# lofcz/Infidex

Measured on AMD Instinct MI355X. Metric: queries/sec, 10M-doc corpus, top-k=20 (whole hot path, index resident in HBM), higher is better.
Workload: dtype f32; 1 GPU; BASELINE config 4: 10000000 docs, vocab 1000000, 1 field(s), 1000-query batches, 2-3-word queries 30% fuzzed, depth 500, top-20; docs=10000000, batch=1000, top_k=20, coverage_depth=500, sessions_in_flight=4, parallelism=single GPU

## Files before the change

### infidex_amd/csrc/infidex_hip.hip

```cpp
#include <type_traits>
#include <cstring>
#include <hip/hip_runtime.h>
#include <stdint.h>
#include <string.h>
#include <stdio.h>
#include <string>
#include <vector>
#include <unordered_map>
#include <algorithm>
#include <map>
#include <mutex>
#include <chrono>
#include <thread>
#include <dlfcn.h>
#include <rccl/rccl.h>
#include "../../include/infidex_hip.h"
#include "unicode_tables.h"

#define WAVE 64
#define FILT_MAXCOL 64

static thread_local std::string g_err;
static int32_t fail(int32_t code, const char* fmt, const char* a = "") {
    char buf[512]; snprintf(buf, sizeof buf, fmt, a); g_err = buf; return code;
}
#define HIPCHK(x) do { hipError_t e_ = (x); if (e_ != hipSuccess) return fail(INFX_EHIP, #x ": %s", hipGetErrorString(e_)); } while (0)
static inline hipError_t enter_device(int device) { const hipError_t e = hipSetDevice(device); (void)hipGetLastError(); return e; }

struct DevIndex {
    int32_t N, T, R, rshift, nRanges, docBase, totalDocs;
    const uint64_t* postOff; const int32_t* postDoc; const uint8_t* postW;
    const float* docNorm;
    const float* docLen;
    const uint8_t* deleted;
    const int64_t* docKey;
    const uint64_t* textOff; const uint16_t* text;
    const uint32_t* skipIdx;
    const uint32_t* skipTbl;
    const uint32_t* psSkip;
    const uint32_t* psSkipTbl;
    const int32_t* wmExact;
    const int32_t* wmLd1;
    const int64_t* docKeyAll;
    int packed;
// ... 483 lines not shown
static hipError_t lds_limit(const void* fn, int device, size_t lds) {
    if (lds <= 64 * 1024) return hipSuccess;
    static std::mutex mu; static std::map<std::pair<int, const void*>, size_t> mark;
    std::lock_guard<std::mutex> lk(mu);
    size_t& hw = mark[{device, fn}];
    if (lds > hw) { const hipError_t e = hipFuncSetAttribute(fn, hipFuncAttributeMaxDynamicSharedMemorySize, (int)lds); if (e != hipSuccess) return e; hw = lds; }
    return hipSuccess;
}

template <int R> static void launch_union(infx_stream* s, uint32_t nv, const uint32_t* dBeg, const uint32_t* dEnd, const int32_t* dMembers, uint32_t* dRangeCount,
                                            const unsigned long long* dBase, int32_t* outDocs) {
    uint64_t blocks = (uint64_t)nv * s->ix->d.nRanges;
    k_union<R><<<dim3((unsigned)blocks), dim3(WAVE), 0, s->st>>>(dev_index(s), dBeg, dEnd, dMembers, nv, dRangeCount, dBase, outDocs);
}
static void launch_union_any(infx_stream* s, uint32_t nv, const uint32_t* dBeg, const uint32_t* dEnd, const int32_t* dMembers, uint32_t* dRangeCount,
                             const unsigned long long* dBase, int32_t* outDocs) {
    switch (s->ix->d.R) {
        case 512: launch_union<512>(s, nv, dBeg, dEnd, dMembers, dRangeCount, dBase, outDocs); break;
        case 1024: launch_union<1024>(s, nv, dBeg, dEnd, dMembers, dRangeCount, dBase, outDocs); break;
        case 2048: launch_union<2048>(s, nv, dBeg, dEnd, dMembers, dRangeCount, dBase, outDocs); break;
        case 4096: launch_union<4096>(s, nv, dBeg, dEnd, dMembers, dRangeCount, dBase, outDocs); break;
        case 8192: launch_union<8192>(s, nv, dBeg, dEnd, dMembers, dRangeCount, dBase, outDocs); break;
        default: launch_union<16384>(s, nv, dBeg, dEnd, dMembers, dRangeCount, dBase, outDocs); break;
    }
}
static bool exact_enabled(const infx_index* ix) { static const bool v = [] { const char* e = getenv("INFX_EXACT"); return !(e && e[0] == '0'); }(); return v && !(ix->cfg.flags & INFX_CFG_NO_EXACT_REPLAY); }
static Arena make_arena(infx_stream* s) {
    return Arena{s->arDoc, s->arScore, s->arCls, s->arMask, s->arExc, (const unsigned long long*)s->dBlockOut, (uint32_t*)s->dBlockOutHi,
                 (uint32_t*)s->dCounts, s->dOverflow, (unsigned long long*)s->dQBytes, (uint32_t*)((unsigned long long*)s->dQBytes + s->lastNqAlloc), (uint2*)s->dDir, s->maskWords};
}
static int acc_stripe() { static const int v = [] { const char* e = getenv("INFX_ACC_STRIPE"); int x = e ? atoi(e) : 0; return (x >= 1 && x <= 64) ? x : 4; }(); return v; }
template <int R> static bool acc_lds_layout_ok() {
    static const bool ok = [] {
        hipFuncAttributes a1{}, a2{}, a4{};
        if (hipFuncGetAttributes(&a1, (const void*)k_accumulate<R, 1>) != hipSuccess || hipFuncGetAttributes(&a2, (const void*)k_accumulate<R, 2>) != hipSuccess ||
            hipFuncGetAttributes(&a4, (const void*)k_accumulate<R, 4>) != hipSuccess) return false;
        return a1.sharedSizeBytes == 0 && a2.sharedSizeBytes == 0 && a4.sharedSizeBytes == 0;
    }();
    return ok;
}
static int acc_sparse_t() { static const int v = [] { const char* e = getenv("INFX_ACC_SPARSE_T"); const int x = e ? atoi(e) : 96; return std::max(0, std::min(4096, x)); }(); return v; }
template <int R> static void launch_acc(infx_stream* s, uint32_t nq, Arena ar, int maxT, int useGrp, int maxRef) {
    (void)maxRef;
    if (!acc_lds_layout_ok<R>()) { s->accLayoutBad = true; return; }
    static const int dbgSkip = [] { const char* e = getenv("INFX_ACC_SKIP"); return e ? atoi(e) : 0; }();
    const int sparseT = s->ix->hPostOff.empty() || s->ix->hPostOff.back() + 4 <= 0xFFFFFFF0ull ? acc_sparse_t() : 0;
    const int stripe = sparseT > 0 ? std::max(1, std::min(4, 65536 / R)) : acc_stripe();
    const int nStripes = (s->ix->d.nRanges + stripe - 1) / stripe;
    const uint64_t blocks = (uint64_t)nq * 8u * ((nStripes + 7) / 8);
    const uint8_t* dense = nullptr;
    if (sparseT > 0) {
        if (grow(s, &s->dDense, &s->capDense, (size_t)nq * nStripes)) { s->accLayoutBad = true; return; }
        hipMemsetAsync(s->dDense, 0, (size_t)nq * nStripes, s->st);
        const size_t sw = (size_t)stripe * (R / 32);
        const int maxTl = (std::min(64, std::max(1, maxT)) + 3) & ~3;
        static const int dbgS = [] { const char* e = getenv("INFX_ACCS_SKIP"); return e ? atoi(e) : 0; }();
        const size_t ldsS = (sw + 64 + 4) * 4 + INFX_NCLASS * 4 + WAVE * 2 + WAVE * 12 + (size_t)WAVE * maxTl + (size_t)64 * maxTl;
#define ACCS_LAUNCH(MW_) k_accumulate_sparse<R, MW_><<<dim3((unsigned)blocks), dim3(WAVE), ldsS, s->st>>>(dev_index(s), (const DevQuery*)s->dQueries, (const DevTerm*)s->dTerms, (const int32_t*)s->dExtra, \
            (const int32_t*)s->dUDocs, (const uint32_t*)s->dURange, nq, ar, stripe, useGrp, (uint8_t*)s->dDense, (uint32_t)sparseT, nStripes, maxTl, dbgS)
        if (ar.maskWords == 4) ACCS_LAUNCH(4); else if (ar.maskWords == 2) ACCS_LAUNCH(2); else ACCS_LAUNCH(1);
#undef ACCS_LAUNCH
        dense = (const uint8_t*)s->dDense;
    }
    const size_t lds = (size_t)R + 128 + ((size_t)(R / 32) + 2) * 4 + INFX_NCLASS * 4 + ACC_CAP_DEFAULT * 2;
#define ACC_LAUNCH(MW_) k_accumulate<R, MW_><<<dim3((unsigned)blocks), dim3(WAVE), lds, s->st>>>(dev_index(s), (const DevQuery*)s->dQueries, (const DevTerm*)s->dTerms, (const int32_t*)s->dExtra, \
        (const int32_t*)s->dUDocs, (const uint32_t*)s->dURange, nq, ar, maxT, stripe, useGrp, dbgSkip, (unsigned long long*)s->dStats, dense, nStripes, \
        s->nAccHeavy != 0xFFFFFFFFu ? (const uint32_t*)s->dAccOrder : nullptr, s->nAccHeavy != 0xFFFFFFFFu ? s->nAccHeavy : 0u)
    if (ar.maskWords == 4) ACC_LAUNCH(4); else if (ar.maskWords == 2) ACC_LAUNCH(2); else ACC_LAUNCH(1);
#undef ACC_LAUNCH
    if (dbgSkip & 8) { unsigned long long h[4] = {0, 0, 0, 0}; hipStreamSynchronize(s->st); hipMemcpy(h, s->dStats, 32, hipMemcpyDeviceToHost); hipMemset(s->dStats, 0, 32);
        fprintf(stderr, "[infx] k_accumulate stats: %llu ranges with candidates (%llu blocks), %.2f rounds/range, %.1f candidates/range\n", h[0], (unsigned long long)blocks, h[0] ? (double)h[1] / h[0] : 0.0, h[0] ? (double)h[2] / h[0] : 0.0); }
}

static const uint32_t* select_order(infx_stream* s, uint32_t nq) {
    static const bool off = [] { const char* e = getenv("INFX_SELECT_LPT"); return e && e[0] == '0'; }();
    if (off || nq < 64 || nq > SEL_ORDER_MAX) return nullptr;
    if (grow(s, &s->dSelOrder, &s->capSelOrder, (size_t)nq * 4)) return nullptr;
    k_select_order<<<1, 1024, 0, s->st>>>((const uint32_t*)s->dBlockOutHi, nq, (uint32_t*)s->dSelOrder);
    return (const uint32_t*)s->dSelOrder;
}
#ifdef SEL_PROF
static void wgprof_dump(const char* name, const unsigned long long* dProf, uint32_t n, const char* const ph[5], hipStream_t st) {
    hipStreamSynchronize(st);
    std::vector<unsigned long long> h((size_t)n * 8); hipMemcpy(h.data(), dProf, h.size() * 8, hipMemcpyDeviceToHost);
    unsigned long long t0 = ~0ull, t5 = 0; for (uint32_t q = 0; q < n; q++) if (h[q * 8]) { t0 = std::min(t0, h[q * 8]); for (int k = 1; k < 6; k++) t5 = std::max(t5, h[q * 8 + k]); }
    fprintf(stderr, "[%s] span %.1f us\n", name, (t5 - t0) / 100.0);
    auto endOf = [&](uint32_t q) { unsigned long long e = h[q * 8]; for (int k = 1; k < 6; k++) e = std::max(e, h[q * 8 + k]); return e; };
    std::vector<uint32_t> ord(n); for (uint32_t q = 0; q < n; q++) ord[q] = q;
    std::sort(ord.begin(), ord.end(), [&](uint32_t a, uint32_t b) { return endOf(a) - h[a * 8] > endOf(b) - h[b * 8]; });
    auto us = [&](uint32_t q, int a, int b) { const unsigned long long x = h[q * 8 + a], y = h[q * 8 + b]; return (x && y) ? (double)(y - x) / 100.0 : -1.0; };
    auto line = [&](const char* tag, uint32_t q) { fprintf(stderr, "[%s] %s wg %u w6 %llu w7 %llu: start %.1f total %.1f | %s %.1f %s %.1f %s %.1f %s %.1f %s %.1f\n", name, tag, q, h[q * 8 + 6], h[q * 8 + 7], (h[q * 8] - t0) / 100.0,
                                                        (endOf(q) - h[q * 8]) / 100.0, ph[0], us(q, 0, 1), ph[1], us(q, 1, 2), ph[2], us(q, 2, 3), ph[3], us(q, 3, 4), ph[4], us(q, 4, 5)); };
    for (int i = 0; i < 10 && i < (int)n; i++) line("top", ord[i]);
    line("p50", ord[n / 2]); line("p90", ord[n / 10]); line("p99", ord[n / 100]);
    std::vector<unsigned long long> en(n); for (uint32_t q = 0; q < n; q++) en[q] = endOf(q) - t0; std::sort(en.begin(), en.end());
    fprintf(stderr, "[%s] ends: p10 %.1f p50 %.1f p90 %.1f p99 %.1f max %.1f us\n", name, en[n / 10] / 100.0, en[n / 2] / 100.0, en[n * 9 / 10] / 100.0, en[n * 99 / 100] / 100.0, en[n - 1] / 100.0);
}
#endif
static uint32_t giant_min_rows() { static const uint32_t v = [] { const char* e = getenv("INFX_SEL_GIANT_MIN"); return e ? (uint32_t)std::max(0, atoi(e)) : 65536u; }(); return v; }
static SelGiant select_giants(infx_stream* s, Arena ar, uint32_t nq, const uint32_t* order) {
    const uint32_t minRows = giant_min_rows();
    SelGiant G{}; if (!order || !minRows || !s->nBoundGiants || s->maxQueryBound < 4ull * minRows) return G;
    const size_t head = (size_t)SELG_MAX * 2 * 4096 * 4 + (size_t)SELG_MAX * 4 * 5, total = head + (size_t)SELG_MAX * SEL_CAP * 8;
    if (grow(s, &s->dSelG, &s->capSelG, total)) return G;
// ... 2376 lines not shown
```

### infidex_amd/csrc/stage1.hip.inc

```

#define F_LOWEST 0x100
#define F_S1 0x200
#define F_S2 0x400
#define CLS_HOLE 0xFF

struct Arena {
    int32_t* doc; float* score; uint8_t* cls;
    unsigned long long* mask;
    uint32_t* exc;
    const unsigned long long* qBase;
    uint32_t* qCursor;
    uint32_t* counts;
    uint32_t* overflow;
    unsigned long long* qBytes;
    uint32_t* qMax;
    uint2* dir;
    int maskWords;
};

#define ACC_WPS 4
#define ACC_PF 2
#define ACC_G 2
#define ACC_CAP_DEFAULT (64 * ACC_G)

typedef int v4i_t __attribute__((ext_vector_type(4)));
typedef const __attribute__((address_space(1))) v4i_t* gint4p;
__device__ __forceinline__ int4 ld4(gint4p p, uint32_t i) { const v4i_t v = p[i]; return make_int4(v.x, v.y, v.z, v.w); }
typedef const __attribute__((address_space(1))) int32_t* gint32p;
__device__ __forceinline__ uint32_t rdl_u(uint32_t v, int l) { return (uint32_t)__builtin_amdgcn_readlane((int)v, l); }
__device__ __forceinline__ float rdl_f(float v, int l) { return __int_as_float(__builtin_amdgcn_readlane(__float_as_int(v), l)); }

typedef __attribute__((address_space(3))) uint8_t lds_u8_t;
#define LDS8(off) (*(lds_u8_t*)(uint32_t)(off))

template <int R, int MW>
__global__ __launch_bounds__(WAVE, ACC_WPS) void k_accumulate(DevIndex ix, const DevQuery* __restrict__ queries,
                                                      const DevTerm* __restrict__ terms, const int32_t* __restrict__ extraDocs,
                                                      const int32_t* __restrict__ unionDocs, const uint32_t* __restrict__ unionRange, uint32_t nq, Arena ar, int maxT, int stripe, int useGrp, int dbgSkip, unsigned long long* __restrict__ stats,
                                                      const uint8_t* __restrict__ dense, int nStripes, const uint32_t* __restrict__ qOrder, uint32_t nHeavy) {
    constexpr int W = R / 32;
    constexpr int WPL = (W + WAVE - 1) / WAVE;
    constexpr int G = ACC_G, CAP = WAVE * ACC_G;
    extern __shared__ __attribute__((aligned(16))) unsigned char smem[];
    uint8_t* sTf = (uint8_t*)smem;
    uint32_t* sBits = (uint32_t*)(sTf + R + 128);
    uint32_t* sHist = sBits + W + 2;
    uint16_t* sDoc = (uint16_t*)(sHist + INFX_NCLASS);

    const int lane = threadIdx.x;
    const uint32_t b = blockIdx.x;
    uint32_t q; int sIdx;
    if (dbgSkip & 32) { q = b % nq; sIdx = (int)(b / nq); }
    else if (qOrder) {
        const uint32_t ns8 = (uint32_t)((nStripes + 7) / 8) * 8u, hb = nHeavy * ns8;
        if (b < hb) { q = qOrder[b / ns8]; sIdx = (int)(b % ns8); }
        else { const uint32_t t = (b - hb) >> 3, nr = nq - nHeavy; q = qOrder[nHeavy + t % nr]; sIdx = (int)((t / nr) * 8u + (b & 7u)); }
    }
    else { const uint32_t t = b >> 3; q = t % nq; sIdx = (int)((t / nq) * 8u + (b & 7u)); }
    if (sIdx * stripe >= ix.nRanges) return;
    if (dense && !dense[(size_t)q * nStripes + (size_t)sIdx]) return;
    const DevQuery Q = queries[q];
    const uint8_t* const del = q_deleted(ix, q);
    const int mode = Q.mode;
    const int nT = (int)Q.numTerms;
    const DevTerm* T = terms + Q.termOff;
    const int nAnd = Q.nAnd;
    const uint32_t Rlane = (uint32_t)R + (uint32_t)lane;
    const unsigned long long qb = ar.qBase[q];
    const uint32_t qcap = (uint32_t)(ar.qBase[q + 1] - qb);
    const int nWin = (nT + WAVE - 1) / WAVE;

    for (int i = lane * 16; i < R + 128; i += WAVE * 16) *(uint4*)(sTf + i) = make_uint4(0, 0, 0, 0);
    for (int i = lane; i < INFX_NCLASS; i += WAVE) sHist[i] = 0;
    unsigned long long myBytes = 0;
    uint32_t myMax = 0;

    uint32_t tApLo = 0, tApHi = 0, tPack = 0, tLen = 0, tMeta = 0, tUpd = 0x1FFu << 16; float tIdf = 0.f;
    uint32_t tRef = 0; bool tGen = false;
    DevTerm tm{}; bool tmValid = false;
    auto load_window_consts = [&](int win) {
        const int t = win * WAVE + lane;
        tmValid = t < nT;
        if (tmValid) tm = T[t];
        tIdf = (tmValid && tm.idf > 0.f) ? tm.idf : 0.f;
        tMeta = tmValid ? (((uint32_t)tm.isVirtual << 16) | ((uint32_t)tm.pad << 24)) : 0u;
        tUpd = 0x1FFu << 16;
        if (tmValid) {
            uint32_t add = 0, rk1 = 0x1FFu;
            if (mode == INFX_MODE_AND) add = ((tm.role & INFX_ROLE_AND) ? 1u : 0u) | ((tm.role & INFX_ROLE_LOWEST) ? F_LOWEST : 0u) | ((tm.role & INFX_ROLE_S1) ? F_S1 : 0u) | ((tm.role & INFX_ROLE_S2) ? F_S2 : 0u);
            else if (mode == INFX_MODE_DISJ && (tm.role & (INFX_ROLE_ELIGIBLE | INFX_ROLE_LOWQ))) rk1 = (uint32_t)tm.rank + 1u;
            tUpd = add | (rk1 << 16);
        }
        tRef = tmValid ? tm.refIdx : 0u;
// ... 273 lines not shown
                        if (pre) cls |= 0x80; else atomicAdd(&sHist[cls], 1u);
                    }
                } else { emit = true; cls = 1; atomicAdd(&sHist[1], 1u); }
            }
            const unsigned long long m = __ballot(emit);
            if (emit) {
                const unsigned long long pos = outBase + written + __popcll(m & ((1ull << lane) - 1));
                ar.doc[pos] = ix.docBase + base + l;
                const float stored = (del && del[ix.docBase + base + l]) ? 0.f : sc;
                ar.score[pos] = stored; myMax = max(myMax, __float_as_uint(stored));
                ar.cls[pos] = cls;
                if (ar.maskWords) {
#pragma unroll
                    for (int w = 0; w < MW; w++) ar.mask[pos * (unsigned long long)MW + w] = cMask[g][w];
                    ar.exc[pos] = cExc[g];
                }
            }
            written += (uint32_t)__popcll(m);
        }
    }
    if (!haveOff || dropped) continue;
    if (lane == 0) { ar.dir[(unsigned long long)q * ix.nRanges + r] = make_uint2(chunkOff, written); myBytes += (unsigned long long)written * 12ull; }
    for (uint32_t i = written + lane; i < ncand; i += WAVE) { ar.cls[outBase + i] = CLS_HOLE; ar.score[outBase + i] = 0.f; }
    }
    for (int i = lane; i < INFX_NCLASS; i += WAVE) { uint32_t c = sHist[i]; if (c) atomicAdd(&ar.counts[(uint64_t)q * INFX_NCLASS + i], c); }
#pragma unroll
    for (int d = 32; d > 0; d >>= 1) myBytes += __shfl_down(myBytes, d);
    if (lane == 0 && myBytes) atomicAdd(&ar.qBytes[q], myBytes);
#pragma unroll
    for (int d = 32; d > 0; d >>= 1) myMax = max(myMax, (uint32_t)__shfl_down((int)myMax, d));
    if (lane == 0 && myMax) atomicMax(&ar.qMax[q], myMax);
}

template <int R>
__global__ __launch_bounds__(WAVE) void k_union(DevIndex ix, const uint32_t* __restrict__ memberBeg, const uint32_t* __restrict__ memberEnd, const int32_t* __restrict__ members,
                                                 uint32_t nv, uint32_t* __restrict__ rangeCount, const unsigned long long* __restrict__ unionBase,
                                                 int32_t* __restrict__ outDocs) {
    constexpr int W = R / 32;
    constexpr int WPL = (W + WAVE - 1) / WAVE;
    __shared__ uint32_t sBits[W];
    __shared__ unsigned long long sBase[WAVE];
    __shared__ uint32_t sLen[WAVE];
    const int lane = threadIdx.x;
    const uint32_t v = blockIdx.x % nv; const int r = (int)(blockIdx.x / nv);
    const int32_t base = r * R, rend = min(base + R, ix.N);
    if (outDocs) { if (r + 1 <= ix.nRanges && rangeCount[(uint64_t)v * (ix.nRanges + 1) + r] == rangeCount[(uint64_t)v * (ix.nRanges + 1) + r + 1]) return; }
    for (int i = lane; i < W; i += WAVE) sBits[i] = 0;
    const uint32_t mb = memberBeg[v], me = memberEnd[v];
    bool any = false;
    for (uint32_t m0 = mb; m0 < me; m0 += WAVE) {
        uint32_t len = 0; unsigned long long b0 = 0;
        if (m0 + lane < me) {
            const int32_t t = members[m0 + lane];
            const uint64_t tb = ix.postOff[t], te = ix.postOff[t + 1];
            const uint32_t sk = ix.skipIdx[t];
            uint32_t lo, hi;
            if (sk != 0xFFFFFFFFu) { lo = ix.skipTbl[sk + r]; hi = ix.skipTbl[sk + r + 1]; }
            else { lo = (uint32_t)(lower_bound_post(ix.postDoc, tb, te, base, ix.packed) - tb); hi = (uint32_t)(lower_bound_post(ix.postDoc, tb + lo, te, rend, ix.packed) - tb); }
            len = hi - lo; b0 = tb + lo;
        }
        sBase[lane] = b0; sLen[lane] = len;
        const int nm = (int)min((uint32_t)WAVE, me - m0);
        for (int k = 0; k < nm; k++) {
            const uint32_t L = sLen[k]; const unsigned long long bb = sBase[k];
            if (L) any = true;
            for (uint32_t i = lane; i < L; i += WAVE) { int l = post_doc(ix.postDoc[bb + i], ix.packed) - base; atomicOr(&sBits[l >> 5], 1u << (l & 31)); }
// ... 393 lines not shown
```

### infidex_amd/csrc/stage1_sparse.hip.inc

```
#define ACCS_U 6

template <int R, int MW>
__global__ __launch_bounds__(WAVE) void k_accumulate_sparse(DevIndex ix, const DevQuery* __restrict__ queries, const DevTerm* __restrict__ terms, const int32_t* __restrict__ extraDocs,
                                                            const int32_t* __restrict__ unionDocs, const uint32_t* __restrict__ unionRange, uint32_t nq, Arena ar, int stripe, int useGrp,
                                                            uint8_t* __restrict__ denseFlag, uint32_t denseT, int nStripes, int maxTl, int dbg) {
    constexpr int U = ACCS_U;
    extern __shared__ __attribute__((aligned(16))) unsigned char smem[];
    const int SW = stripe * (R / 32);
    const int WPL = max(1, SW / WAVE);
    const int wsh = 31 - __clz(WPL);
    const int SWP = (SW + (SW >> wsh) + 3) & ~3;
    uint32_t* sBits = (uint32_t*)smem;
    uint32_t* sHist = sBits + SWP;
    uint16_t* sDoc = (uint16_t*)(sHist + INFX_NCLASS);
    uint2* sTA = (uint2*)(sDoc + WAVE);
    uint32_t* sTL = (uint32_t*)(sTA + WAVE);
    uint8_t* sHit = (uint8_t*)(sTL + WAVE);
    uint32_t* sSamp = (uint32_t*)(sHit + (size_t)WAVE * maxTl);

    const int lane = threadIdx.x;
    const uint32_t b = blockIdx.x;
    const uint32_t bt = b >> 3; const uint32_t q = bt % nq; const int sIdx = (int)((bt / nq) * 8u + (b & 7u));
    const int r0 = sIdx * stripe;
    if (r0 >= ix.nRanges) return;
    const int rEnd = min(ix.nRanges, r0 + stripe), nr = rEnd - r0;
    const int32_t base = r0 * R;
    const int32_t send = min(rEnd * R, ix.N);
    const uint32_t span = (uint32_t)(send - base);
    const DevQuery Q = queries[q];
    const uint8_t* const del = q_deleted(ix, q);
    const int mode = Q.mode;
    const int nT = (int)Q.numTerms;
    const DevTerm* T = terms + Q.termOff;
    const int nAnd = Q.nAnd;
    const unsigned long long qb = ar.qBase[q];
    const uint32_t qcap = (uint32_t)(ar.qBase[q + 1] - qb);
    const int nWin = (nT + WAVE - 1) / WAVE;
    const unsigned long long lt = (1ull << lane) - 1;
    unsigned long long myBytes = 0;

    uint32_t tApLo = 0, tApHi = 0, tLen = 0, tMeta = 0, tUpd = 0x1FFu << 16; float tIdf = 0.f;
    auto load_window = [&](int win) -> bool {
        const int t = win * WAVE + lane;
        tLen = 0; tApLo = 0; tApHi = 0; tIdf = 0.f; tMeta = 0; tUpd = 0x1FFu << 16;
        bool gen = false;
        if (t < nT) {
            const DevTerm tm = T[t];
            tIdf = tm.idf > 0.f ? tm.idf : 0.f;
            uint32_t add = 0, rk1 = 0x1FFu;
            if (mode == INFX_MODE_AND) {
                add = ((tm.role & INFX_ROLE_AND) ? 1u : 0u) | ((tm.role & INFX_ROLE_LOWEST) ? F_LOWEST : 0u) | ((tm.role & INFX_ROLE_S1) ? F_S1 : 0u) | ((tm.role & INFX_ROLE_S2) ? F_S2 : 0u);
                gen = (tm.role & (INFX_ROLE_S1 | INFX_ROLE_S2)) != 0;
            } else if (mode == INFX_MODE_DISJ && (tm.role & (INFX_ROLE_ELIGIBLE | INFX_ROLE_LOWQ))) { rk1 = (uint32_t)tm.rank + 1u; gen = true; }
            tUpd = add | (rk1 << 16);
            tMeta = (uint32_t)tm.isVirtual | ((uint32_t)tm.pad << 8) | ((uint32_t)tm.refIdx << 16);
            uint32_t lo, hi;
            if (tm.isVirtual & 4) { lo = unionRange[tm.skip + r0]; hi = unionRange[tm.skip + rEnd]; }
            else if (tm.skip != 0xFFFFFFFFu) { lo = ix.skipTbl[tm.skip + r0]; hi = ix.skipTbl[tm.skip + rEnd]; }
            else {
                const int32_t* arr = (tm.isVirtual & 1) ? extraDocs : ix.postDoc;
                const int pk = (tm.isVirtual & 5) ? 0 : ix.packed;
                lo = (uint32_t)(lower_bound_post(arr, tm.begin, tm.end, base, pk) - tm.begin);
                hi = (uint32_t)(lower_bound_post(arr, tm.begin + lo, tm.end, send, pk) - tm.begin);
            }
            tLen = hi - lo;
            const int32_t* dp = ((tm.isVirtual & 4) ? unionDocs : ((tm.isVirtual & 1) ? extraDocs : ix.postDoc)) + (tm.begin + lo);
            const unsigned long long ap = (unsigned long long)(uintptr_t)dp;
            tApLo = (uint32_t)ap; tApHi = (uint32_t)(ap >> 32);
            myBytes += (unsigned long long)tLen * (tm.isVirtual ? 4u : 5u);
        }
        return gen;
    };

    unsigned long long psBase = 0; uint32_t psLen = 0;
    if (Q.prefixSet >= 0) {
        const uint64_t pb = ix.psOff[Q.prefixSet], pe = ix.psOff[Q.prefixSet + 1];
        const uint32_t sk = ix.psSkip[Q.prefixSet];
        uint64_t lo, hi;
        if (sk != 0xFFFFFFFFu) { lo = pb + ix.psSkipTbl[sk + r0]; hi = pb + ix.psSkipTbl[sk + rEnd]; }
        else { lo = lower_bound_i32(ix.psDocs, pb, pe, base); hi = lower_bound_i32(ix.psDocs, lo, pe, send); }
        psBase = lo; psLen = (uint32_t)(hi - lo);
    }
    bool anyGen = (mode == INFX_MODE_PREFIX) && psLen > 0;
    bool bitsClear = false;
    auto set_bit = [&](uint32_t l) { const uint32_t w = l >> 5; atomicOr(&sBits[w + (w >> wsh)], 1u << (l & 31)); };
    auto clear_bits = [&]() { if (!bitsClear) { for (int i = lane * 4; i < SWP; i += WAVE * 4) *(uint4*)(sBits + i) = make_uint4(0, 0, 0, 0); bitsClear = true; } };
    if (mode == INFX_MODE_PREFIX) {
        if (psLen > denseT) { if (lane == 0) denseFlag[(size_t)q * nStripes + sIdx] = 1; return; }
        if (nWin == 1) load_window(0);
        if (anyGen) { clear_bits(); for (uint32_t i = lane; i < psLen; i += WAVE) set_bit((uint32_t)(ix.psDocs[psBase + i] - base)); }
    } else {
        for (int win = 0; win < nWin; win++) {
            const bool gen = load_window(win);
            if (__ballot(gen && tLen > denseT)) { if (lane == 0) denseFlag[(size_t)q * nStripes + sIdx] = 1; return; }
            unsigned long long gm = __ballot(gen && tLen > 0);
            if (gm) { anyGen = true; clear_bits(); }
            while (gm) {
                const int tl = __ffsll((long long)gm) - 1; gm &= gm - 1;
                const uint32_t len = rdl_u(tLen, tl), iv = rdl_u(tMeta, tl) & 0xFFu;
                const unsigned long long ap = ((unsigned long long)rdl_u(tApHi, tl) << 32) | rdl_u(tApLo, tl);
                const int pk = (iv & 5) ? 0 : ix.packed;
                if (!(iv & 1)) {
                    const uint32_t mis = (uint32_t)((ap >> 2) & 3u);
                    const gint4p ap4 = (gint4p)(uintptr_t)(ap - 4ull * mis);
                    const uint32_t total = len + mis;
                    for (uint32_t i = (uint32_t)lane * 4u; i < total; i += 4u * WAVE) {
                        const int4 c = ld4(ap4, i >> 2);
                        const uint32_t l0 = (uint32_t)post_doc(c.x, pk) - (uint32_t)base, l1 = (uint32_t)post_doc(c.y, pk) - (uint32_t)base;
                        const uint32_t l2 = (uint32_t)post_doc(c.z, pk) - (uint32_t)base, l3 = (uint32_t)post_doc(c.w, pk) - (uint32_t)base;
                        if (l0 < span) set_bit(l0);
                        if (l1 < span) set_bit(l1);
                        if (l2 < span) set_bit(l2);
                        if (l3 < span) set_bit(l3);
                    }
                } else {
                    const gint32p dp = (gint32p)(uintptr_t)ap;
                    for (uint32_t i = lane; i < len; i += WAVE) set_bit((uint32_t)(post_doc(dp[i], pk) - base));
                }
            }
        }
    }
    uint32_t ncand = 0, cnt = 0, incl = 0;
    if (anyGen) {
        for (int j = 0; j < WPL; j++) { const int wi = lane * WPL + j; if (wi < SW) cnt += __popc(sBits[wi + lane]); }
        incl = cnt;
#pragma unroll
        for (int d = 1; d < WAVE; d <<= 1) { const uint32_t v = __shfl_up(incl, d); if (lane >= d) incl += v; }
        ncand = rdl_u(incl, WAVE - 1);
    }
    if (ncand > denseT) {
        if (lane == 0) denseFlag[(size_t)q * nStripes + sIdx] = 1;
        return;
    }
    if (dbg & 2) ncand = 0;
    if (ncand) {
        for (int i = lane; i < INFX_NCLASS; i += WAVE) sHist[i] = 0;
        uint32_t chunkOffV = 0;
        if (lane == 0) chunkOffV = atomicAdd(&ar.qCursor[q], ncand);
        uint32_t chunkOff = 0; unsigned long long outBase = 0; bool haveOff = false, dropped = false;
        uint32_t written = 0, rCnt = 0, myMax = 0;
        for (uint32_t rb = 0; rb < ncand && !dropped; rb += WAVE) {
        const uint32_t nslot = min((uint32_t)WAVE, ncand - rb);
        {
            uint32_t sl = incl - cnt;
            if (sl < rb + nslot && incl > rb)
                for (int j = 0; j < WPL; j++) {
                    const int wi = lane * WPL + j;
                    uint32_t bits = wi < SW ? sBits[wi + lane] : 0u;
                    while (bits) { const int bpos = __ffs(bits) - 1; bits &= bits - 1; const uint32_t rel = sl - rb; if (rel < nslot) sDoc[rel] = (uint16_t)(wi * 32 + bpos); sl++; }
                }
        }
        const bool valid = (uint32_t)lane < nslot;
        const uint32_t cDoc = valid ? (uint32_t)sDoc[lane] : 0u;
        const uint32_t docS = (uint32_t)base + cDoc;
        const float cNorm = valid ? ix.docNorm[docS] : 1.0f;
        float cAcc = 0.f; uint32_t cFlag = 0, cRank = 0x1FFu, cGrp = 0, cExc = 0; unsigned long long cMask[MW];
#pragma unroll
        for (int w = 0; w < MW; w++) cMask[w] = 0ull;

        struct TermS { uint32_t meta, upd; float idf; };
        auto apply = [&](const TermS& S, uint32_t tfb) {
            const uint32_t iv = S.meta & 0xFFu, grp = (S.meta >> 8) & 0xFFu, ref = S.meta >> 16;
            const bool unit = iv != 0;
            if (!__ballot(tfb != 0)) return;
            if (grp && useGrp) { const bool dup = cGrp == grp; if (tfb) cGrp = grp; if (dup) tfb = 0; }
            const bool hit = tfb != 0;
            {
                const float tf = unit ? 1.0f : (float)tfb;
                const float denom = tf + cNorm;
                const float core = (tf * (1.2f + 1.0f)) / denom;
                const float sc = S.idf * (core + 1.0f);
                cAcc += hit ? sc : 0.f;
            }
            const uint32_t addFlag = S.upd & 0xFFFFu, rk1 = S.upd >> 16;
            cFlag += hit ? addFlag : 0u;
            cRank = min(cRank, hit ? rk1 : 0x1FFu);
            if (ar.maskWords != 0 && ref < 32u * (uint32_t)MW) {
                const uint32_t capCode = unit ? 1u : 3u;
                const unsigned long long code = (unsigned long long)min(tfb, capCode) << ((ref & 31u) * 2u);
                const uint32_t wsel = ref >> 5;
#pragma unroll
                for (int w = 0; w < MW; w++) if (wsel == (uint32_t)w) cMask[w] |= code;
                if (!unit && __ballot(tfb >= 3u)) {
                    const uint32_t rec = ((ref + 1u) << 8) | tfb;
                    if (tfb >= 3u) { if (!(cExc & 0xFFFFu)) cExc |= rec; else if (!(cExc >> 16)) cExc |= rec << 16; }
                }
            }
        };
        const uint32_t tpp = (uint32_t)WAVE / nslot;
        const uint32_t mdiv = (65536u + nslot - 1u) / nslot;
        const uint32_t kl = ((uint32_t)lane * mdiv) >> 16, cl = (uint32_t)lane - kl * nslot;
        const uint32_t pairDoc = (uint32_t)base + (uint32_t)sDoc[cl < nslot ? cl : 0];
        for (int win = 0; win < nWin; win++) {
            if (nWin > 1) load_window(win);
            const unsigned long long tmask = __ballot(tLen > 0);
            if (!tmask) continue;
            const uint32_t nLive = (uint32_t)__popcll(tmask);
            if (tLen > 0) {
                const uint32_t k = (uint32_t)__popcll(tmask & lt), iv = tMeta & 0xFFu;
                sTA[k] = make_uint2(tApLo, tApHi); sTL[k] = tLen | ((iv & 5u) ? 1u << 29 : 0u);
            }
            for (uint32_t i = (uint32_t)lane * 4u; i < nLive * (uint32_t)WAVE; i += 4u * WAVE) *(uint32_t*)(sHit + i) = 0u;
            for (uint32_t i = (uint32_t)lane; i < nLive * 16u; i += WAVE) {
                const uint32_t k = i >> 4, j = i & 15u;
                const uint2 a = sTA[k]; const uint32_t len = sTL[k] & 0x1FFFFFFFu;
                sSamp[i] = ((const uint32_t*)(uintptr_t)(((unsigned long long)a.y << 32) | a.x))[(j * len) >> 4];
            }
            const uint32_t keyP = ix.packed ? ((pairDoc << 8) | 0xFFu) : pairDoc;
            const uint32_t* const pd = (const uint32_t*)ix.postDoc;
            for (uint32_t k0 = 0; k0 < nLive && !(dbg & 1); k0 += tpp * (uint32_t)U) {
                uint32_t n[U], pos[U], xb[U];
#pragma unroll
                for (int u = 0; u < U; u++) {
                    const uint32_t kk = k0 + (uint32_t)u * tpp + kl;
                    n[u] = 0; pos[u] = 0; xb[u] = 0xFFFFFFFFu;
                    if (kl < tpp && kk < nLive) {
                        const uint32_t L = sTL[kk];
                        if (!((L >> 29) & 1u)) {
                            const uint2 a = sTA[kk];
                            const uint32_t A = (uint32_t)((const uint32_t*)(uintptr_t)(((unsigned long long)a.y << 32) | a.x) - pd), len = L & 0x1FFFFFFFu;
                            const uint32_t* sp = sSamp + kk * 16u;
                            uint32_t j = 0;
#pragma unroll
                            for (uint32_t st = 8; st > 0; st >>= 1) j += (sp[j + st] <= keyP) ? st : 0u;
                            const uint32_t lo = (j * len) >> 4, hi = j == 15u ? len : (((j + 1u) * len) >> 4);
                            pos[u] = A + lo; n[u] = max(hi - lo, 1u); xb[u] = sp[j];
                        }
                    }
                }
                bool more = false;
#pragma unroll
                for (int u = 0; u < U; u++) more = more || n[u] > 1;
                while (__ballot(more)) {
                    uint32_t o[U], x[U];
#pragma unroll
                    for (int u = 0; u < U; u++) { const uint32_t half = n[u] >> 1; o[u] = pos[u] + half; x[u] = (n[u] > 1) ? pd[o[u]] : xb[u]; n[u] -= half; }
                    more = false;
#pragma unroll
                    for (int u = 0; u < U; u++) { const bool le = x[u] <= keyP; pos[u] = le ? o[u] : pos[u]; xb[u] = le ? x[u] : xb[u]; more = more || n[u] > 1; }
                }
#pragma unroll
                for (int u = 0; u < U; u++) {
                    if (ix.packed ? (xb[u] >> 8) == pairDoc : xb[u] == pairDoc) {
                        const uint32_t tfb = ix.packed ? (xb[u] & 0xFFu) : (uint32_t)ix.postW[pos[u]];
                        sHit[(k0 + (uint32_t)u * tpp + kl) * (uint32_t)WAVE + cl] = (uint8_t)tfb;
                    }
                }
            }
            for (unsigned long long lm = (dbg & 1) ? 0ull : __ballot((uint32_t)lane < nLive && ((sTL[lane] >> 29) & 1u)); lm; lm &= lm - 1) {
                const uint32_t kL = (uint32_t)__ffsll((long long)lm) - 1u;
                const uint2 a = sTA[kL]; const uint32_t len = sTL[kL] & 0x1FFFFFFFu;
                const uint32_t* lp = (const uint32_t*)(uintptr_t)(((unsigned long long)a.y << 32) | a.x);
                if (valid) {
                    uint32_t lo = 0, hi = len;
                    while (lo < hi) { const uint32_t m = (lo + hi) >> 1; if (lp[m] < docS) lo = m + 1u; else hi = m; }
                    if (lo < len && lp[lo] == docS) sHit[kL * (uint32_t)WAVE + (uint32_t)lane] = (uint8_t)1u;
                }
            }
            uint32_t k = 0;
            for (unsigned long long tm = (dbg & 4) ? 0ull : tmask; tm; tm &= tm - 1, k++) {
                const int tl = __ffsll((long long)tm) - 1;
                TermS S; S.meta = rdl_u(tMeta, tl); S.upd = rdl_u(tUpd, tl); S.idf = rdl_f(tIdf, tl);
                apply(S, valid ? (uint32_t)sHit[k * (uint32_t)WAVE + (uint32_t)lane] : 0u);
            }
        }
        if (!haveOff) {
            chunkOff = (uint32_t)rfl_i((int)chunkOffV); haveOff = true;
            if (chunkOff + ncand > qcap) { if (lane == 0) atomicExch(ar.overflow, 1u); dropped = true; }
            outBase = qb + chunkOff;
        }
        if (!dropped) {
            bool emit = false; uint8_t cls = 0; const float sc = cAcc; const uint32_t f = (mode == INFX_MODE_DISJ) ? (cRank == 0x1FFu ? 0u : cRank) : cFlag;
            if (valid && sc > 0.f) {
                if (mode == INFX_MODE_AND) {
                    if (f & (F_S1 | F_S2)) {
                        emit = true;
                        const int c2 = (int)(f & 0xFF);
                        const bool t1 = c2 == nAnd - 1;
                        const bool t0b = t1 && (f & F_LOWEST);
                        cls = (uint8_t)((t0b ? 1 : 0) | ((t1 && nAnd >= 3) ? 2 : 0) | ((f & F_S1) ? 4 : 0) | ((f & F_S2) ? 8 : 0));
                        atomicAdd(&sHist[cls], 1u);
                    }
                } else if (mode == INFX_MODE_DISJ) {
                    if (f != 0) {
                        emit = true;
                        cls = (uint8_t)((f - 1) & 0x7F);
                        bool pre = false;
                        if (psLen) {
                            const int32_t d = (int32_t)docS;
                            const uint64_t p = lower_bound_i32(ix.psDocs, psBase, psBase + psLen, d);
                            pre = p < psBase + psLen && ix.psDocs[p] == d;
                        }
                        if (pre) cls |= 0x80; else atomicAdd(&sHist[cls], 1u);
                    }
                } else { emit = true; cls = 1; atomicAdd(&sHist[1], 1u); }
            }
            const unsigned long long m = __ballot(emit);
// ... 1 lines not shown
                const unsigned long long pos = outBase + written + __popcll(m & lt);
                ar.doc[pos] = ix.docBase + (int32_t)docS;
                const float stored = (del && del[ix.docBase + (int32_t)docS]) ? 0.f : sc;
                ar.score[pos] = stored; myMax = max(myMax, __float_as_uint(stored));
                ar.cls[pos] = cls;
                if (ar.maskWords) {
#pragma unroll
                    for (int w = 0; w < MW; w++) ar.mask[pos * (unsigned long long)MW + w] = cMask[w];
                    ar.exc[pos] = cExc;
                }
            }
            written += (uint32_t)__popcll(m);
            const uint32_t rng = cDoc / (uint32_t)R;
#pragma unroll 1
            for (int k = 0; k < nr; k++) { const uint32_t c = (uint32_t)__popcll(__ballot(emit && rng == (uint32_t)k)); if (lane == k) rCnt += c; }
        }
        }
        if (haveOff && !dropped) {
            uint32_t rIncl = rCnt;
#pragma unroll
            for (int d = 1; d < WAVE; d <<= 1) { const uint32_t v = __shfl_up(rIncl, d); if (lane >= d) rIncl += v; }
            if (lane < nr && rCnt) ar.dir[(unsigned long long)q * ix.nRanges + r0 + lane] = make_uint2(chunkOff + rIncl - rCnt, rCnt);
            if (lane == 0) myBytes += (unsigned long long)written * 12ull;
            for (uint32_t i = written + lane; i < ncand; i += WAVE) { ar.cls[outBase + i] = CLS_HOLE; ar.score[outBase + i] = 0.f; }
            for (int i = lane; i < INFX_NCLASS; i += WAVE) { const uint32_t c = sHist[i]; if (c) atomicAdd(&ar.counts[(uint64_t)q * INFX_NCLASS + i], c); }
#pragma unroll
            for (int d = 32; d > 0; d >>= 1) myMax = max(myMax, (uint32_t)__shfl_down((int)myMax, d));
            if (lane == 0 && myMax) atomicMax(&ar.qMax[q], myMax);
        }
    }
#pragma unroll
    for (int d = 32; d > 0; d >>= 1) myBytes += __shfl_down(myBytes, d);
    if (lane == 0 && myBytes) atomicAdd(&ar.qBytes[q], myBytes);
}
```

Measured before the change: 96080 queries/s.

## Merge sparse and streaming accumulate into one launch with in-block fallback

Adds k_accumulate_merged, which runs the sparse accumulation body and, when a stripe turns out dense, falls through to the streaming body in the same block. The dense-flag buffer, its memset, and the second kernel launch that re-reads it are no longer needed. The term-table LDS size is capped so occupancy matches the streaming kernel, and windows with too many live terms are handed to the streaming path. The cost is a heavier combined kernel whose register pressure could lower occupancy, plus possible extra streaming work when the cap forces a fallback. Wave barriers were also added inside the sparse body.

```diff
diff --git a/infidex_amd/csrc/infidex_hip.hip b/infidex_amd/csrc/infidex_hip.hip
--- a/infidex_amd/csrc/infidex_hip.hip
+++ b/infidex_amd/csrc/infidex_hip.hip
@@ -10,6 +10,7 @@
 #include <algorithm>
 #include <map>
 #include <mutex>
+#include <atomic>
 #include <chrono>
 #include <thread>
 #include <dlfcn.h>
@@ -559,44 +560,82 @@
 static int acc_stripe() { static const int v = [] { const char* e = getenv("INFX_ACC_STRIPE"); int x = e ? atoi(e) : 0; return (x >= 1 && x <= 64) ? x : 4; }(); return v; }
 template <int R> static bool acc_lds_layout_ok() {
     static const bool ok = [] {
-        hipFuncAttributes a1{}, a2{}, a4{};
-        if (hipFuncGetAttributes(&a1, (const void*)k_accumulate<R, 1>) != hipSuccess || hipFuncGetAttributes(&a2, (const void*)k_accumulate<R, 2>) != hipSuccess ||
-            hipFuncGetAttributes(&a4, (const void*)k_accumulate<R, 4>) != hipSuccess) return false;
-        return a1.sharedSizeBytes == 0 && a2.sharedSizeBytes == 0 && a4.sharedSizeBytes == 0;
+        const void* const k[6] = {(const void*)k_accumulate<R, 1>, (const void*)k_accumulate<R, 2>, (const void*)k_accumulate<R, 4>,
+                                  (const void*)k_accumulate_merged<R, 1>, (const void*)k_accumulate_merged<R, 2>, (const void*)k_accumulate_merged<R, 4>};
+        for (const void* f : k) { hipFuncAttributes a{}; if (hipFuncGetAttributes(&a, f) != hipSuccess || a.sharedSizeBytes != 0) return false; }
+        return true;
     }();
     return ok;
 }
 static int acc_sparse_t() { static const int v = [] { const char* e = getenv("INFX_ACC_SPARSE_T"); const int x = e ? atoi(e) : 96; return std::max(0, std::min(4096, x)); }(); return v; }
+static bool acc_merged() { static const bool v = [] { const char* e = getenv("INFX_ACC_MERGED"); return !(e && e[0] == '0'); }(); return v; }
+static size_t acc_sparse_lds(int R, int stripe, int maxTl) {
+    return ((size_t)stripe * (R / 32) + 64 + 4) * 4 + INFX_NCLASS * 4 + WAVE * 2 + WAVE * 12 + (size_t)WAVE * maxTl + (size_t)64 * maxTl;
+}
+template <int R, int MW> static int acc_merged_max_tl(int stripe, size_t ldsStream) {
+    static const int cap = [&] {
+        int nStream = 0, n = 0;
+        if (hipOccupancyMaxActiveBlocksPerMultiprocessor(&nStream, (const void*)k_accumulate<R, MW>, WAVE, ldsStream) != hipSuccess || nStream <= 0) return 0;
+        for (int tl = 64; tl >= 4; tl -= 4)
+            if (hipOccupancyMaxActiveBlocksPerMultiprocessor(&n, (const void*)k_accumulate_merged<R, MW>, WAVE, std::max(ldsStream, acc_sparse_lds(R, stripe, tl))) == hipSuccess && n >= nStream) return tl;
+        return 0;
+    }();
+    return cap;
+}
 template <int R> static void launch_acc(infx_stream* s, uint32_t nq, Arena ar, int maxT, int useGrp, int maxRef) {
     (void)maxRef;
     if (!acc_lds_layout_ok<R>()) { s->accLayoutBad = true; return; }
     static const int dbgSkip = [] { const char* e = getenv("INFX_ACC_SKIP"); return e ? atoi(e) : 0; }();
+    static const int dbgS = [] { const char* e = getenv("INFX_ACCS_SKIP"); return e ? atoi(e) : 0; }();
+    static const bool dbgPrint = getenv("INFX_DEBUG") != nullptr;
     const int sparseT = s->ix->hPostOff.empty() || s->ix->hPostOff.back() + 4 <= 0xFFFFFFF0ull ? acc_sparse_t() : 0;
     const int stripe = sparseT > 0 ? std::max(1, std::min(4, 65536 / R)) : acc_stripe();
     const int nStripes = (s->ix->d.nRanges + stripe - 1) / stripe;
     const uint64_t blocks = (uint64_t)nq * 8u * ((nStripes + 7) / 8);
+    const size_t lds = (size_t)R + 128 + ((size_t)(R / 32) + 2) * 4 + INFX_NCLASS * 4 + ACC_CAP_DEFAULT * 2;
+    const uint32_t* const qOrder = s->nAccHeavy != 0xFFFFFFFFu ? (const uint32_t*)s->dAccOrder : nullptr;
+    const uint32_t nHeavy = s->nAccHeavy != 0xFFFFFFFFu ? s->nAccHeavy : 0u;
+    const int maxTl = (std::min(64, std::max(1, maxT)) + 3) & ~3;
     const uint8_t* dense = nullptr;
-    if (sparseT > 0) {
+    int schedule = 0, tlUsed = 0;
+    if (sparseT > 0 && acc_merged() && !(dbgSkip & 32)) {
+        const int capTl = ar.maskWords == 4 ? acc_merged_max_tl<R, 4>(stripe, lds) : ar.maskWords == 2 ? acc_merged_max_tl<R, 2>(stripe, lds) : acc_merged_max_tl<R, 1>(stripe, lds);
+        if (capTl > 0) {
+            schedule = 1; tlUsed = std::min(maxTl, capTl);
+            const size_t ldsM = std::max(lds, acc_sparse_lds(R, stripe, tlUsed));
+#define ACCM_LAUNCH(MW_) k_accumulate_merged<R, MW_><<<dim3((unsigned)blocks), dim3(WAVE), ldsM, s->st>>>(dev_index(s), (const DevQuery*)s->dQueries, (const DevTerm*)s->dTerms, (const int32_t*)s->dExtra, \
+                (const int32_t*)s->dUDocs, (const uint32_t*)s->dURange, nq, ar, stripe, useGrp, dbgSkip, (unsigned long long*)s->dStats, (uint32_t)sparseT, nStripes, tlUsed, dbgS, qOrder, nHeavy)
+            if (ar.maskWords == 4) ACCM_LAUNCH(4); else if (ar.maskWords == 2) ACCM_LAUNCH(2); else ACCM_LAUNCH(1);
+#undef ACCM_LAUNCH
+        }
+    }
+    if (sparseT > 0 && schedule == 0) {
+        schedule = 2; tlUsed = maxTl;
         if (grow(s, &s->dDense, &s->capDense, (size_t)nq * nStripes)) { s->accLayoutBad = true; return; }
         hipMemsetAsync(s->dDense, 0, (size_t)nq * nStripes, s->st);
-        const size_t sw = (size_t)stripe * (R / 32);
-        const int maxTl = (std::min(64, std::max(1, maxT)) + 3) & ~3;
-        static const int dbgS = [] { const char* e = getenv("INFX_ACCS_SKIP"); return e ? atoi(e) : 0; }();
-        const size_t ldsS = (sw + 64 + 4) * 4 + INFX_NCLASS * 4 + WAVE * 2 + WAVE * 12 + (size_t)WAVE * maxTl + (size_t)64 * maxTl;
+        const size_t ldsS = acc_sparse_lds(R, stripe, maxTl);
 #define ACCS_LAUNCH(MW_) k_accumulate_sparse<R, MW_><<<dim3((unsigned)blocks), dim3(WAVE), ldsS, s->st>>>(dev_index(s), (const DevQuery*)s->dQueries, (const DevTerm*)s->dTerms, (const int32_t*)s->dExtra, \
             (const int32_t*)s->dUDocs, (const uint32_t*)s->dURange, nq, ar, stripe, useGrp, (uint8_t*)s->dDense, (uint32_t)sparseT, nStripes, maxTl, dbgS)
         if (ar.maskWords == 4) ACCS_LAUNCH(4); else if (ar.maskWords == 2) ACCS_LAUNCH(2); else ACCS_LAUNCH(1);
 #undef ACCS_LAUNCH
         dense = (const uint8_t*)s->dDense;
     }
-    const size_t lds = (size_t)R + 128 + ((size_t)(R / 32) + 2) * 4 + INFX_NCLASS * 4 + ACC_CAP_DEFAULT * 2;
+    if (schedule != 1) {
 #define ACC_LAUNCH(MW_) k_accumulate<R, MW_><<<dim3((unsigned)blocks), dim3(WAVE), lds, s->st>>>(dev_index(s), (const DevQuery*)s->dQueries, (const DevTerm*)s->dTerms, (const int32_t*)s->dExtra, \
-        (const int32_t*)s->dUDocs, (const uint32_t*)s->dURange, nq, ar, maxT, stripe, useGrp, dbgSkip, (unsigned long long*)s->dStats, dense, nStripes, \
-        s->nAccHeavy != 0xFFFFFFFFu ? (const uint32_t*)s->dAccOrder : nullptr, s->nAccHeavy != 0xFFFFFFFFu ? s->nAccHeavy : 0u)
-    if (ar.maskWords == 4) ACC_LAUNCH(4); else if (ar.maskWords == 2) ACC_LAUNCH(2); else ACC_LAUNCH(1);
+            (const int32_t*)s->dUDocs, (const uint32_t*)s->dURange, nq, ar, maxT, stripe, useGrp, dbgSkip, (unsigned long long*)s->dStats, dense, nStripes, qOrder, nHeavy)
+        if (ar.maskWords == 4) ACC_LAUNCH(4); else if (ar.maskWords == 2) ACC_LAUNCH(2); else ACC_LAUNCH(1);
 #undef ACC_LAUNCH
-    if (dbgSkip & 8) { unsigned long long h[4] = {0, 0, 0, 0}; hipStreamSynchronize(s->st); hipMemcpy(h, s->dStats, 32, hipMemcpyDeviceToHost); hipMemset(s->dStats, 0, 32);
-        fprintf(stderr, "[infx] k_accumulate stats: %llu ranges with candidates (%llu blocks), %.2f rounds/range, %.1f candidates/range\n", h[0], (unsigned long long)blocks, h[0] ? (double)h[1] / h[0] : 0.0, h[0] ? (double)h[2] / h[0] : 0.0); }
+    }
+    if (dbgPrint) {
+        static std::atomic<int> last{-1};
+        const int key = (schedule * 8 + ar.maskWords) * 256 + tlUsed;
+        if (last.exchange(key) != key)
+            fprintf(stderr, "[infx] accumulate: %s, R %d, stripe %d, mask words %d, maxT %d, sparse tables for %d slices per window (a window of this batch holds up to %d)\n",
+                    schedule == 1 ? "one merged launch" : schedule == 2 ? "two launches (sparse, streaming)" : "the streaming kernel alone", R, stripe, ar.maskWords, maxT, tlUsed, maxTl);
+    }
+    if (dbgSkip & 8) { unsigned long long h[5] = {0, 0, 0, 0, 0}; hipStreamSynchronize(s->st); hipMemcpy(h, s->dStats, 40, hipMemcpyDeviceToHost); hipMemset(s->dStats, 0, 40);
+        fprintf(stderr, "[infx] k_accumulate stats: %llu ranges with candidates (%llu blocks), %.2f rounds/range, %.1f candidates/range; merged launch: %llu stripes finished sparse, %llu handed to the streaming body\n",
+                h[0], (unsigned long long)blocks, h[0] ? (double)h[1] / h[0] : 0.0, h[0] ? (double)h[2] / h[0] : 0.0, h[3], h[4]); }
 }
 
 static const uint32_t* select_order(infx_stream* s, uint32_t nq) {
diff --git a/infidex_amd/csrc/stage1.hip.inc b/infidex_amd/csrc/stage1.hip.inc
--- a/infidex_amd/csrc/stage1.hip.inc
+++ b/infidex_amd/csrc/stage1.hip.inc
@@ -33,32 +33,30 @@
 typedef __attribute__((address_space(3))) uint8_t lds_u8_t;
 #define LDS8(off) (*(lds_u8_t*)(uint32_t)(off))
 
+__device__ __forceinline__ void acc_block_map(const uint32_t b, const uint32_t nq, const int nStripes, const uint32_t* __restrict__ qOrder, const uint32_t nHeavy, const bool queryFastest,
+                                              uint32_t& q, int& sIdx) {
+    if (queryFastest) { q = b % nq; sIdx = (int)(b / nq); }
+    else if (qOrder) {
+        const uint32_t ns8 = (uint32_t)((nStripes + 7) / 8) * 8u, hb = nHeavy * ns8;
+        if (b < hb) { q = qOrder[b / ns8]; sIdx = (int)(b % ns8); }
+        else { const uint32_t t = (b - hb) >> 3, nr = nq - nHeavy; q = qOrder[nHeavy + t % nr]; sIdx = (int)((t / nr) * 8u + (b & 7u)); }
+    }
+    else { const uint32_t t = b >> 3; q = t % nq; sIdx = (int)((t / nq) * 8u + (b & 7u)); }
+}
+
 template <int R, int MW>
-__global__ __launch_bounds__(WAVE, ACC_WPS) void k_accumulate(DevIndex ix, const DevQuery* __restrict__ queries,
-                                                      const DevTerm* __restrict__ terms, const int32_t* __restrict__ extraDocs,
-                                                      const int32_t* __restrict__ unionDocs, const uint32_t* __restrict__ unionRange, uint32_t nq, Arena ar, int maxT, int stripe, int useGrp, int dbgSkip, unsigned long long* __restrict__ stats,
-                                                      const uint8_t* __restrict__ dense, int nStripes, const uint32_t* __restrict__ qOrder, uint32_t nHeavy) {
+__device__ __forceinline__ void acc_stream_body(const DevIndex& ix, const DevQuery* __restrict__ queries, const DevTerm* __restrict__ terms, const int32_t* __restrict__ extraDocs,
+                                                const int32_t* __restrict__ unionDocs, const uint32_t* __restrict__ unionRange, const Arena& ar, const int stripe, const int useGrp,
+                                                const int dbgSkip, unsigned long long* __restrict__ stats, const uint32_t q, const int sIdx, unsigned char* smem) {
     constexpr int W = R / 32;
     constexpr int WPL = (W + WAVE - 1) / WAVE;
     constexpr int G = ACC_G, CAP = WAVE * ACC_G;
-    extern __shared__ __attribute__((aligned(16))) unsigned char smem[];
     uint8_t* sTf = (uint8_t*)smem;
     uint32_t* sBits = (uint32_t*)(sTf + R + 128);
     uint32_t* sHist = sBits + W + 2;
     uint16_t* sDoc = (uint16_t*)(sHist + INFX_NCLASS);
 
     const int lane = threadIdx.x;
-    const uint32_t b = blockIdx.x;
-    uint32_t q; int sIdx;
-    if (dbgSkip & 32) { q = b % nq; sIdx = (int)(b / nq); }
-    else if (qOrder) {
-        const uint32_t ns8 = (uint32_t)((nStripes + 7) / 8) * 8u, hb = nHeavy * ns8;
-        if (b < hb) { q = qOrder[b / ns8]; sIdx = (int)(b % ns8); }
-        else { const uint32_t t = (b - hb) >> 3, nr = nq - nHeavy; q = qOrder[nHeavy + t % nr]; sIdx = (int)((t / nr) * 8u + (b & 7u)); }
-    }
-    else { const uint32_t t = b >> 3; q = t % nq; sIdx = (int)((t / nq) * 8u + (b & 7u)); }
-    if (sIdx * stripe >= ix.nRanges) return;
-    if (dense && !dense[(size_t)q * nStripes + (size_t)sIdx]) return;
     const DevQuery Q = queries[q];
     const uint8_t* const del = q_deleted(ix, q);
     const int mode = Q.mode;
@@ -398,6 +396,19 @@
     if (lane == 0 && myMax) atomicMax(&ar.qMax[q], myMax);
 }
 
+template <int R, int MW>
+__global__ __launch_bounds__(WAVE, ACC_WPS) void k_accumulate(DevIndex ix, const DevQuery* __restrict__ queries,
+                                                      const DevTerm* __restrict__ terms, const int32_t* __restrict__ extraDocs,
+                                                      const int32_t* __restrict__ unionDocs, const uint32_t* __restrict__ unionRange, uint32_t nq, Arena ar, int maxT, int stripe, int useGrp, int dbgSkip, unsigned long long* __restrict__ stats,
+                                                      const uint8_t* __restrict__ dense, int nStripes, const uint32_t* __restrict__ qOrder, uint32_t nHeavy) {
+    extern __shared__ __attribute__((aligned(16))) unsigned char smem[];
+    uint32_t q; int sIdx;
+    acc_block_map(blockIdx.x, nq, nStripes, qOrder, nHeavy, (dbgSkip & 32) != 0, q, sIdx);
+    if (sIdx * stripe >= ix.nRanges) return;
+    if (dense && !dense[(size_t)q * nStripes + (size_t)sIdx]) return;
+    acc_stream_body<R, MW>(ix, queries, terms, extraDocs, unionDocs, unionRange, ar, stripe, useGrp, dbgSkip, stats, q, sIdx, smem);
+}
+
 template <int R>
 __global__ __launch_bounds__(WAVE) void k_union(DevIndex ix, const uint32_t* __restrict__ memberBeg, const uint32_t* __restrict__ memberEnd, const int32_t* __restrict__ members,
                                                  uint32_t nv, uint32_t* __restrict__ rangeCount, const unsigned long long* __restrict__ unionBase,
diff --git a/infidex_amd/csrc/stage1_sparse.hip.inc b/infidex_amd/csrc/stage1_sparse.hip.inc
--- a/infidex_amd/csrc/stage1_sparse.hip.inc
+++ b/infidex_amd/csrc/stage1_sparse.hip.inc
@@ -1,11 +1,10 @@
 #define ACCS_U 6
 
 template <int R, int MW>
-__global__ __launch_bounds__(WAVE) void k_accumulate_sparse(DevIndex ix, const DevQuery* __restrict__ queries, const DevTerm* __restrict__ terms, const int32_t* __restrict__ extraDocs,
-                                                            const int32_t* __restrict__ unionDocs, const uint32_t* __restrict__ unionRange, uint32_t nq, Arena ar, int stripe, int useGrp,
-                                                            uint8_t* __restrict__ denseFlag, uint32_t denseT, int nStripes, int maxTl, int dbg) {
+__device__ __forceinline__ bool acc_sparse_body(const DevIndex& ix, const DevQuery* __restrict__ queries, const DevTerm* __restrict__ terms, const int32_t* __restrict__ extraDocs,
+                                                const int32_t* __restrict__ unionDocs, const uint32_t* __restrict__ unionRange, const Arena& ar, const int stripe, const int useGrp,
+                                                const uint32_t denseT, const int maxTl, const int dbg, const uint32_t q, const int sIdx, unsigned char* smem) {
     constexpr int U = ACCS_U;
-    extern __shared__ __attribute__((aligned(16))) unsigned char smem[];
     const int SW = stripe * (R / 32);
     const int WPL = max(1, SW / WAVE);
     const int wsh = 31 - __clz(WPL);
@@ -19,10 +18,7 @@
     uint32_t* sSamp = (uint32_t*)(sHit + (size_t)WAVE * maxTl);
 
     const int lane = threadIdx.x;
-    const uint32_t b = blockIdx.x;
-    const uint32_t bt = b >> 3; const uint32_t q = bt % nq; const int sIdx = (int)((bt / nq) * 8u + (b & 7u));
     const int r0 = sIdx * stripe;
-    if (r0 >= ix.nRanges) return;
     const int rEnd = min(ix.nRanges, r0 + stripe), nr = rEnd - r0;
     const int32_t base = r0 * R;
     const int32_t send = min(rEnd * R, ix.N);
@@ -86,13 +82,15 @@
     auto set_bit = [&](uint32_t l) { const uint32_t w = l >> 5; atomicOr(&sBits[w + (w >> wsh)], 1u << (l & 31)); };
     auto clear_bits = [&]() { if (!bitsClear) { for (int i = lane * 4; i < SWP; i += WAVE * 4) *(uint4*)(sBits + i) = make_uint4(0, 0, 0, 0); bitsClear = true; } };
     if (mode == INFX_MODE_PREFIX) {
-        if (psLen > denseT) { if (lane == 0) denseFlag[(size_t)q * nStripes + sIdx] = 1; return; }
-        if (nWin == 1) load_window(0);
+        if (psLen > denseT) return true;
+        if (nWin > 1 && maxTl < WAVE) return true;
+        if (nWin == 1) { load_window(0); if (__popcll(__ballot(tLen > 0)) > maxTl) return true; }
         if (anyGen) { clear_bits(); for (uint32_t i = lane; i < psLen; i += WAVE) set_bit((uint32_t)(ix.psDocs[psBase + i] - base)); }
     } else {
         for (int win = 0; win < nWin; win++) {
             const bool gen = load_window(win);
-            if (__ballot(gen && tLen > denseT)) { if (lane == 0) denseFlag[(size_t)q * nStripes + sIdx] = 1; return; }
+            if (__ballot(gen && tLen > denseT)) return true;
+            if (__popcll(__ballot(tLen > 0)) > maxTl) return true;
             unsigned long long gm = __ballot(gen && tLen > 0);
             if (gm) { anyGen = true; clear_bits(); }
             while (gm) {
@@ -128,10 +126,7 @@
         for (int d = 1; d < WAVE; d <<= 1) { const uint32_t v = __shfl_up(incl, d); if (lane >= d) incl += v; }
         ncand = rdl_u(incl, WAVE - 1);
     }
-    if (ncand > denseT) {
-        if (lane == 0) denseFlag[(size_t)q * nStripes + sIdx] = 1;
-        return;
-    }
+    if (ncand > denseT) return true;
     if (dbg & 2) ncand = 0;
     if (ncand) {
         for (int i = lane; i < INFX_NCLASS; i += WAVE) sHist[i] = 0;
@@ -150,6 +145,7 @@
                     while (bits) { const int bpos = __ffs(bits) - 1; bits &= bits - 1; const uint32_t rel = sl - rb; if (rel < nslot) sDoc[rel] = (uint16_t)(wi * 32 + bpos); sl++; }
                 }
         }
+        __builtin_amdgcn_wave_barrier();
         const bool valid = (uint32_t)lane < nslot;
         const uint32_t cDoc = valid ? (uint32_t)sDoc[lane] : 0u;
         const uint32_t docS = (uint32_t)base + cDoc;
@@ -200,12 +196,14 @@
                 const uint32_t k = (uint32_t)__popcll(tmask & lt), iv = tMeta & 0xFFu;
                 sTA[k] = make_uint2(tApLo, tApHi); sTL[k] = tLen | ((iv & 5u) ? 1u << 29 : 0u);
             }
+            __builtin_amdgcn_wave_barrier();
             for (uint32_t i = (uint32_t)lane * 4u; i < nLive * (uint32_t)WAVE; i += 4u * WAVE) *(uint32_t*)(sHit + i) = 0u;
             for (uint32_t i = (uint32_t)lane; i < nLive * 16u; i += WAVE) {
                 const uint32_t k = i >> 4, j = i & 15u;
                 const uint2 a = sTA[k]; const uint32_t len = sTL[k] & 0x1FFFFFFFu;
                 sSamp[i] = ((const uint32_t*)(uintptr_t)(((unsigned long long)a.y << 32) | a.x))[(j * len) >> 4];
             }
+            __builtin_amdgcn_wave_barrier();
             const uint32_t keyP = ix.packed ? ((pairDoc << 8) | 0xFFu) : pairDoc;
             const uint32_t* const pd = (const uint32_t*)ix.postDoc;
             for (uint32_t k0 = 0; k0 < nLive && !(dbg & 1); k0 += tpp * (uint32_t)U) {
@@ -247,6 +245,7 @@
                     }
                 }
             }
+            __builtin_amdgcn_wave_barrier();
             for (unsigned long long lm = (dbg & 1) ? 0ull : __ballot((uint32_t)lane < nLive && ((sTL[lane] >> 29) & 1u)); lm; lm &= lm - 1) {
                 const uint32_t kL = (uint32_t)__ffsll((long long)lm) - 1u;
                 const uint2 a = sTA[kL]; const uint32_t len = sTL[kL] & 0x1FFFFFFFu;
@@ -257,12 +256,14 @@
                     if (lo < len && lp[lo] == docS) sHit[kL * (uint32_t)WAVE + (uint32_t)lane] = (uint8_t)1u;
                 }
             }
+            __builtin_amdgcn_wave_barrier();
             uint32_t k = 0;
             for (unsigned long long tm = (dbg & 4) ? 0ull : tmask; tm; tm &= tm - 1, k++) {
                 const int tl = __ffsll((long long)tm) - 1;
                 TermS S; S.meta = rdl_u(tMeta, tl); S.upd = rdl_u(tUpd, tl); S.idf = rdl_f(tIdf, tl);
                 apply(S, valid ? (uint32_t)sHit[k * (uint32_t)WAVE + (uint32_t)lane] : 0u);
             }
+            __builtin_amdgcn_wave_barrier();
         }
         if (!haveOff) {
             chunkOff = (uint32_t)rfl_i((int)chunkOffV); haveOff = true;
@@ -330,4 +331,32 @@
 #pragma unroll
     for (int d = 32; d > 0; d >>= 1) myBytes += __shfl_down(myBytes, d);
     if (lane == 0 && myBytes) atomicAdd(&ar.qBytes[q], myBytes);
+    return false;
 }
+
+template <int R, int MW>
+__global__ __launch_bounds__(WAVE) void k_accumulate_sparse(DevIndex ix, const DevQuery* __restrict__ queries, const DevTerm* __restrict__ terms, const int32_t* __restrict__ extraDocs,
+                                                            const int32_t* __restrict__ unionDocs, const uint32_t* __restrict__ unionRange, uint32_t nq, Arena ar, int stripe, int useGrp,
+                                                            uint8_t* __restrict__ denseFlag, uint32_t denseT, int nStripes, int maxTl, int dbg) {
+    extern __shared__ __attribute__((aligned(16))) unsigned char smem[];
+    const uint32_t b = blockIdx.x;
+    const uint32_t bt = b >> 3; const uint32_t q = bt % nq; const int sIdx = (int)((bt / nq) * 8u + (b & 7u));
+    if (sIdx * stripe >= ix.nRanges) return;
+    if (acc_sparse_body<R, MW>(ix, queries, terms, extraDocs, unionDocs, unionRange, ar, stripe, useGrp, denseT, maxTl, dbg, q, sIdx, smem) && threadIdx.x == 0)
+        denseFlag[(size_t)q * nStripes + sIdx] = 1;
+}
+
+template <int R, int MW>
+__global__ __launch_bounds__(WAVE, ACC_WPS) void k_accumulate_merged(DevIndex ix, const DevQuery* __restrict__ queries, const DevTerm* __restrict__ terms, const int32_t* __restrict__ extraDocs,
+                                                                     const int32_t* __restrict__ unionDocs, const uint32_t* __restrict__ unionRange, uint32_t nq, Arena ar, int stripe, int useGrp,
+                                                                     int dbgSkip, unsigned long long* __restrict__ stats, uint32_t denseT, int nStripes, int maxTl, int dbgS,
+                                                                     const uint32_t* __restrict__ qOrder, uint32_t nHeavy) {
+    extern __shared__ __attribute__((aligned(16))) unsigned char smem[];
+    uint32_t q; int sIdx;
+    acc_block_map(blockIdx.x, nq, nStripes, qOrder, nHeavy, false, q, sIdx);
+    if (sIdx * stripe >= ix.nRanges) return;
+    const bool dense = acc_sparse_body<R, MW>(ix, queries, terms, extraDocs, unionDocs, unionRange, ar, stripe, useGrp, denseT, maxTl, dbgS, q, sIdx, smem);
+    if ((dbgSkip & 8) && threadIdx.x == 0) atomicAdd(&stats[dense ? 4 : 3], 1ull);
+    if (!dense) return;
+    acc_stream_body<R, MW>(ix, queries, terms, extraDocs, unionDocs, unionRange, ar, stripe, useGrp, dbgSkip, stats, q, sIdx, smem);
+}
```

Measured after the change: 95670 queries/s. Within noise of the previous version (-0.4%).
